# lionnus/I-ViT

Measured on AMD Instinct MI355X. Metric: images/sec DeiT-B INT8 @batch256, 1→8 MI355X; % INT8 MFMA peak, higher is better.
Workload: dtype int8; 1 GPU; DeiT-B INT8 integer-only forward, batch 256 per GPU, 224x224; global_batch=256, parallelism=dp1, launch=hip-graph replay, bitwidth=8, activation_ranges=power-of-two, operators=I-ViT (IVITIntLayerNorm, Shiftmax, ShiftGELU)

## Files before the change

i-vit_amd/csrc/check_resources.py:

```python
#!/usr/bin/env python3
import re
import sys

GUARDED = ("gemm_i8_wreg_kernel", "gemm_i8_pers_kernel")
FIELDS = {"VGPRs": r"\bVGPRs: (\d+)", "AGPRs": r"AGPRs: (\d+)", "Scratch": r"ScratchSize \[bytes/lane\]: (\d+)",
          "Occupancy": r"Occupancy \[waves/SIMD\]: (\d+)", "VGPRSpill": r"VGPRs Spill: (\d+)", "SGPRSpill": r"SGPRs Spill: (\d+)",
          "LDS": r"LDS Size \[bytes/block\]: (\d+)"}


def parse(text):
    kernels, cur = {}, None
    for line in text.splitlines():
        m = re.search(r"Function Name: (\S+)", line)
        if m:
            cur = kernels.setdefault(m.group(1), {})
            continue
        if cur is None:
            continue
        for k, pat in FIELDS.items():
            m = re.search(pat, line)
            if m and k not in cur:
                cur[k] = int(m.group(1))
    return kernels


def occupancy_rules(path, what):
    kernels = parse(open(path, errors="replace").read())
    bad, seen = [], 0
    for name, r in sorted(kernels.items()):
        if what == "attention" and "attention_long_kernel" in name:
            m = re.search(r"attention_long_kernelILi(\d+)ELb([01])ELi(\d+)ELi(\d+)E", name)
            occ, need_no_scratch = int(m.group(4)) // 256, True
        elif what == "attention" and "attention_cls_kernel" in name:
            occ, need_no_scratch = 3, True
        elif what == "attention":
            m = re.search(r"attention_kernelILi(\d+)ELi(\d+)ELi(\d+)ELb([01])E", name)
            if not m:
                continue
            occ, need_no_scratch = int(m.group(3)), m.group(4) == "0"
        elif what == "swin":
            if "window_attention_long_kernel" in name:
                occ, need_no_scratch = 2, True
            elif "window_attention_kernel" in name:
                occ, need_no_scratch = 4, True
            else:
                m = re.search(r"layernorm_i16_i8_tiled(_compat)?_kernelILi(\d+)ELi(\d+)E", name)
                if not m:
                    continue
                occ, need_no_scratch = (3 if m.group(1) and int(m.group(3)) >= 2 else 4), True
        elif "head_topk_kernel" in name:
            occ, need_no_scratch = 8, True
        else:
            m = re.search(r"layernorm_i8_stream_kernelILi(\d+)ELi(\d+)ELi(\d+)ELb([01])ELi(\d+)E", name)
            if not m:
                continue
            occ = int(m.group(5))
            need_no_scratch = m.group(4) == "0" or int(m.group(2)) == 3
        seen += 1
        ok = r.get("Occupancy", 0) >= occ and (r.get("Scratch") == 0 and r.get("VGPRSpill", 0) == 0 or not need_no_scratch)
        print(("ok   " if ok else "FAIL ") + f"{name}: VGPR {r.get('VGPRs')}, scratch {r.get('Scratch')}, occupancy {r.get('Occupancy')} (launcher assumes {occ}"
              f"{', no scratch' if need_no_scratch else ''})")
        if not ok:
            bad.append(name)
    if seen == 0:
        print("check_resources: no", what, "kernel found in", path)
        return 1
    if bad:
        print("check_resources: occupancy / scratch assumption of the launchers violated:", ", ".join(bad))
        return 1
    return 0


def main(path):
    kernels = parse(open(path, errors="replace").read())
    bad, seen = [], 0
    for name, r in sorted(kernels.items()):
        if not any(g in name for g in GUARDED):
            continue
        seen += 1
        regs = r.get("VGPRs", 0) + r.get("AGPRs", 0)
        line = (f"{name}: VGPR+AGPR {regs}, scratch {r.get('Scratch')}, VGPR spill {r.get('VGPRSpill')}, "
                f"SGPR spill {r.get('SGPRSpill')}, occupancy {r.get('Occupancy')}, LDS {r.get('LDS')}")
        ok = (r.get("Scratch") == 0 and r.get("VGPRSpill") == 0 and regs <= 256 and r.get("Occupancy", 0) >= 2
              and r.get("LDS", 0) <= 81920)
        print(("ok   " if ok else "FAIL ") + line)
        if not ok:
            bad.append(name)
    if seen == 0:
        print("check_resources: no guarded kernel found in", path)
        return 1
    if bad:
        print("check_resources: register / scratch budget of the inline-asm GEMM kernels violated:", ", ".join(bad))
        return 1
    return 0


if __name__ == "__main__":
    sys.exit(occupancy_rules(sys.argv[1], sys.argv[2]) if len(sys.argv) > 2 else main(sys.argv[1]))
```

i-vit_amd/csrc/gemm.hip:

```cpp
#include <type_traits>
#include "gemm_common.h"

namespace {

template <int EPI>
__global__ __launch_bounds__(NT) void gemm_i8_kernel(GemmArgs g)
{
    __shared__ __attribute__((aligned(16))) char smem[SMEM_BYTES + BN * 8];

    const int nblk = g.tiles_m * g.tiles_n;
    const int bid = blockIdx.x;
    const int q8 = nblk >> 3, r8 = nblk & 7, xcd = bid & 7;
    const int lid = (xcd < r8 ? xcd * (q8 + 1) : r8 * (q8 + 1) + (xcd - r8) * q8) + (bid >> 3);
    const int tm = lid / g.tiles_n, tn = lid - tm * g.tiles_n;
    const int m0 = tm * BM, n0 = tn * BN;

    const int tid = threadIdx.x;
    const int lane = tid & 63, wave = tid >> 6;
    const int wm = wave >> 1, wn = wave & 1;
    const int h = lane >> 5, l31 = lane & 31;
    if constexpr (EPI != EPI_I32 && EPI != EPI_RQ16 && EPI != EPI_RQ16_RES16) fill_rq_table(g, smem + SMEM_BYTES, n0, BN, tid);

    const int srow = tid >> 2, sc = tid & 3;
    const int8_t* ap[2];
// ... 862 lines not shown
                acc[ii] = *reinterpret_cast<const v4i*>(bias + 16 * i + 4 * g4);
#pragma unroll
                for (int ks = 0; ks < SK_MAXK / 32; ++ks)
                    if (ks < nks)
                        acc[ii] = __builtin_amdgcn_mfma_i32_16x16x32_i8(*reinterpret_cast<const long*>(smem + ((size_t)(i * nks + ks) * 64 + lane) * 8),
                                                                         bf[ks], acc[ii], 0, 0, 0);
            }
            int b[4][4];
            unsigned unc = 0;
#pragma unroll
            for (int ii = 0; ii < 4; ++ii) {
                const int i = min(i0 + ii, nsub - 1);
#pragma unroll
                for (int r = 0; r < 4; ++r) {
                    const float2 lh = lohi[16 * i + 4 * g4 + r];
                    const float a = (float)acc[ii][r];
                    const int tl = __float_as_int(__builtin_fmaf(a, lh.x, 12582912.0f));
                    const int th = __float_as_int(__builtin_fmaf(a, lh.y, 12582912.0f));
                    asm("v_sad_u32 %0, %1, %2, %3" : "=v"(unc) : "v"(tl), "v"(th), "v"(unc));
                    b[ii][r] = clamp_i32(tl, 0x4B400000 - 128, 0x4B400000 + 127);
                }
            }
            if (__builtin_amdgcn_ballot_w64(unc != 0) != 0) {
#pragma unroll
                for (int ii = 0; ii < 4; ++ii) {
                    const int c0 = 16 * min(i0 + ii, nsub - 1) + 4 * g4;
#pragma unroll
                    for (int r = 0; r < 4; ++r) {
                        const double tq = (double)acc[ii][r] * dyadic_mult(g.m[c0 + r], g.e[c0 + r]) + IVIT_MAGIC;
                        b[ii][r] = clamp_i32((int)(unsigned)__double_as_longlong(tq), -128, 127);
                    }
                }
            }
            unsigned D[4];
#pragma unroll
            for (int ii = 0; ii < 4; ++ii)
                D[ii] = __builtin_amdgcn_perm((unsigned)b[ii][1], (unsigned)b[ii][0], 0x0c0c0400u) |
                        __builtin_amdgcn_perm((unsigned)b[ii][3], (unsigned)b[ii][2], 0x04000c0cu);
            typedef unsigned v2u __attribute__((ext_vector_type(2)));
            const v2u ab = __builtin_amdgcn_permlane32_swap(D[0], D[2], false, false);
            const v2u cd = __builtin_amdgcn_permlane32_swap(D[1], D[3], false, false);
            const v2u ac = __builtin_amdgcn_permlane16_swap(ab.x, cd.x, false, false);
            const v2u bd = __builtin_amdgcn_permlane16_swap(ab.y, cd.y, false, false);
            const int ci = i0 + g4;
            if (ci < nsub && t < g.M) {
                const int4 v = make_int4((int)ac.x, (int)ac.y, (int)bd.x, (int)bd.y);
                if constexpr (EPI == EPI_QKV) *reinterpret_cast<int4*>(out + coff[4 * ci] + qrow_off) = v;
                else *reinterpret_cast<int4*>(out + (int64_t)t * g.ldo + 16 * ci) = v;
            }
        }
    }
}

template <int EPI>
int launch_gemm(GemmArgs& g, const char* name, ivit_stream_t stream, int qkv_planes = 3)
{
    IVIT_REQUIRE(g.A && g.W && g.out, "%s: NULL operand", name);
    IVIT_REQUIRE(g.M > 0 && g.N > 0 && g.K > 0, "%s: empty problem M=%d N=%d K=%d", name, g.M, g.N, g.K);
    IVIT_REQUIRE(g.K % BK == 0, "%s: K=%d must be a multiple of %d", name, g.K, BK);
    IVIT_REQUIRE(g.lda >= g.K && g.ldw >= g.K && g.lda % 16 == 0 && g.ldw % 16 == 0,
                 "%s: lda=%lld ldw=%lld must be >= K and multiples of 16", name, (long long)g.lda, (long long)g.ldw);
    IVIT_REQUIRE(((uintptr_t)g.A % 16 == 0) && ((uintptr_t)g.W % 16 == 0) && ((uintptr_t)g.out % 16 == 0),
                 "%s: operands must be 16-byte aligned", name);
    if (EPI == EPI_I32 || EPI == EPI_RQ16 || EPI == EPI_RQ16_RES16) {
        IVIT_REQUIRE(g.N % 4 == 0 && g.ldo % 4 == 0 && g.ldo >= g.N, "%s: N=%d ldo=%lld must be multiples of 4", name,
                     g.N, (long long)g.ldo);
        if (EPI == EPI_RQ16 || EPI == EPI_RQ16_RES16)
            IVIT_REQUIRE(g.m && g.e && ((uintptr_t)g.m % 16 == 0) && ((uintptr_t)g.e % 16 == 0) && ((uintptr_t)g.out % 8 == 0),
                         "%s: requantiser tables missing or misaligned", name);
    } else {
        IVIT_REQUIRE(g.m && g.e, "%s: NULL requantiser table", name);
        IVIT_REQUIRE(((uintptr_t)g.bias % 16 == 0), "%s: bias must be 16-byte aligned", name);
        IVIT_REQUIRE(g.N % 16 == 0, "%s: N=%d must be a multiple of 16", name, g.N);
        IVIT_REQUIRE(((uintptr_t)g.m % 16 == 0) && ((uintptr_t)g.e % 16 == 0), "%s: m/e tables must be 16-byte aligned",
                     name);
    }
    if (EPI == EPI_RQ || EPI == EPI_RESID)
        IVIT_REQUIRE(g.ldo >= g.N && g.ldo % 16 == 0, "%s: ldo=%lld must be >= N and a multiple of 16", name,
                     (long long)g.ldo);
    if (EPI == EPI_RESID)
        IVIT_REQUIRE(g.res && g.ldr >= g.N && g.ldr % 16 == 0 && ((uintptr_t)g.res % 16 == 0),
                     "%s: residual operand missing or misaligned", name);
    if (EPI == EPI_RESID16 || EPI == EPI_RQ16_RES16)
        IVIT_REQUIRE(g.res && g.ldr >= g.N && g.ldr % 8 == 0 && ((uintptr_t)g.res % 16 == 0) && g.ldo >= g.N && g.ldo % 8 == 0,
                     "%s: 16-bit residual / output rows must be 16-byte aligned (ld multiples of 8 elements)", name);
    if (EPI == EPI_QKV) {
        IVIT_REQUIRE(g.tokens > 0 && g.heads > 0 && g.head_dim > 0 && g.head_dim % 16 == 0,
                     "%s: bad head geometry tokens=%d heads=%d head_dim=%d", name, g.tokens, g.heads, g.head_dim);
        IVIT_REQUIRE((int64_t)g.M * g.N < 2147483648ll, "%s: q/k/v output of %lld bytes exceeds the 2 GiB the 32-bit head-major offsets cover",
                     name, (long long)g.M * g.N);
        IVIT_REQUIRE(g.N == qkv_planes * g.heads * g.head_dim && g.M % g.tokens == 0,
                     "%s: N=%d != %d*heads*head_dim or M=%d %% tokens=%d != 0", name, g.N, qkv_planes, g.M, g.tokens);
    }
#if IVIT_LAB
    g.stamp = reinterpret_cast<unsigned long long*>(g_stamp_buf);
#endif
    const bool blocks = g.a_blocks || g.w_blocks;
    if constexpr (EPI == EPI_RQ || EPI == EPI_QKV) {
        if (!blocks && !g.w_frags && !g.out_blocks && !g.lut && g.M >= 8192 && g.K >= 32 && g.K <= SK_MAXK && g.K % 32 == 0 && g.N >= 16 &&
            g.N <= SK_MAXN && g.N % 16 == 0 && g.lda % 16 == 0 && g.ldw % 8 == 0 && ((uintptr_t)g.A % 16 == 0) && ((uintptr_t)g.W % 8 == 0) &&
            ((uintptr_t)g.out % 16 == 0) && (EPI == EPI_QKV || g.ldo % 16 == 0) && (EPI != EPI_QKV || g.head_dim % 16 == 0) && (int64_t)g.M * (EPI == EPI_QKV ? g.N : g.ldo) < 4294967296ll &&
            !g_force_small && !(IVIT_LAB && (g_debug_flags2 & (1 << 20)))) {
            const int nstrips = (g.M + 15) >> 4;
            const int grid = (nstrips + SK_WPB - 1) / SK_WPB < 512 ? (nstrips + SK_WPB - 1) / SK_WPB : 512;
            const bool any_k = IVIT_LAB && (g_debug_flags2 & (1 << 21));
            if (g.K == 128 && !any_k) hipLaunchKernelGGL((gemm_i8_skinny_kernel<EPI, 4>), dim3(grid), dim3(SK_NT), 0, ivit_stream(stream), g);
// ... 40 lines not shown
                    default: break;
                }
            }
#endif
            if (g.w_frags == 2) {
                if constexpr (EPI != EPI_RQ16_RES16) {
                    IVIT_REQUIRE(((int64_t)g.M + 16) * (EPI == EPI_QKV ? g.N : g.ldo) < 4294967296ll &&
                                     (EPI != EPI_RESID || ((int64_t)g.M + 16) * g.ldr < 4294967296ll),
                                 "%s: IVIT_W_FRAGS16 addresses its output (and residual) with 32-bit offsets: operand of 4 GiB or more", name);
#if IVIT_LAB
                    if constexpr (EPI == EPI_RQ || EPI == EPI_RESID) {
                        if ((g_debug_flags2 & 256) && g.stamp) {
                            if (EPI == EPI_RESID && g.res_f32) hipLaunchKernelGGL((gemm_i8_wreg_kernel<EPI, 16 | 2048 | 4096, true>), grid, dim3(BIG_NT), 0, ivit_stream(stream), g);
                            else hipLaunchKernelGGL((gemm_i8_wreg_kernel<EPI, 16 | 2048, true>), grid, dim3(BIG_NT), 0, ivit_stream(stream), g);
                            IVIT_CHECK_LAUNCH(name);
                        }
                    }
#endif
                    if constexpr (EPI == EPI_RESID) {
                        if (g.res_f32) {
                            hipLaunchKernelGGL((gemm_i8_wreg_kernel<EPI, 4096, true>), grid, dim3(BIG_NT), 0, ivit_stream(stream), g);
                            IVIT_CHECK_LAUNCH(name);
                        }
                    }
                    hipLaunchKernelGGL((gemm_i8_wreg_kernel<EPI, 0, true>), grid, dim3(BIG_NT), 0, ivit_stream(stream), g);
                    IVIT_CHECK_LAUNCH(name);
                } else {
                    IVIT_REQUIRE(false, "%s: IVIT_W_FRAGS16 has no 16-bit epilogue; pack the weights with ivit_pack_weight_frags_i8", name);
                }
            }
            hipLaunchKernelGGL((gemm_i8_wreg_kernel<EPI>), grid, dim3(BIG_NT), 0, ivit_stream(stream), g);
            IVIT_CHECK_LAUNCH(name);
        }
    }
    if constexpr (EPI != EPI_I32 && EPI != EPI_RQ16 && EPI != EPI_RQ16_RES16) {
        if (g.M >= 2048 && g.N >= BCH && !g_force_small) {
            g.stagger = (g_debug_flags & 64) ? 0 : 512;
            g.tiles_m = (g.M + BTOK - 1) / BTOK;
            g.tiles_n = (g.N + BCH - 1) / BCH;
            const int ntiles = g.tiles_m * g.tiles_n;
            const bool one_per_cu = (g_debug_flags & 4096) != 0;
            const int SLOTS = (one_per_cu || (g_debug_flags & 67108864)) ? 256 : 512;
            const int rounds = ntiles / SLOTS, R = ntiles - rounds * SLOTS;
            const bool split = R > 0 && !(g_debug_flags & 134217728) &&
                               ((g_debug_flags & 2048) ? 2 * R <= SLOTS : 2 * R <= 256) && !one_per_cu;
            g.split_from = split ? rounds * SLOTS : ntiles;
            g.cu_turns = (g_debug_flags & 32768) ? 1 : 0;
            g.stagger_units = (g_debug_flags >> 16) & 63;
            const int grid = rounds > 0 ? SLOTS : (split ? 2 * R : R);
            hipLaunchKernelGGL((gemm_i8_pers_kernel<EPI>), dim3(grid), dim3(BIG_NT), one_per_cu ? 20480 : 0, ivit_stream(stream), g);
            IVIT_CHECK_LAUNCH(name);
        }
    }
    g.tiles_m = (g.M + BM - 1) / BM;
    g.tiles_n = (g.N + BN - 1) / BN;
    hipLaunchKernelGGL(gemm_i8_kernel<EPI>, dim3(g.tiles_m * g.tiles_n), dim3(NT), 0, ivit_stream(stream), g);
    IVIT_CHECK_LAUNCH(name);
}

__global__ __launch_bounds__(256) void pack_weight_frags_kernel(const int8_t* W, int64_t ldw, int N, int K, int8_t* dst)
{
    const int c16 = K >> 4, n64 = (N + 63) & ~63;
    const int64_t total = (int64_t)n64 * c16;
    for (int64_t q = (int64_t)blockIdx.x * 256 + threadIdx.x; q < total; q += (int64_t)gridDim.x * 256) {
        const int n = (int)(q / c16), k = (int)(q - (int64_t)n * c16) << 4;
        int4 v = make_int4(0, 0, 0, 0);
        if (n < N) v = *reinterpret_cast<const int4*>(W + (int64_t)n * ldw + k);
        const int64_t off = ((int64_t)(n >> 6) * (K >> 6) + (k >> 6)) * 4096 + ((((n >> 5) & 1) * 2 + ((k >> 5) & 1)) * 2 + ((k >> 4) & 1)) * 512 + (n & 31) * 16;
        *reinterpret_cast<int4*>(dst + off) = v;
    }
}

__global__ __launch_bounds__(256) void pack_weight_frags16_kernel(const int8_t* W, int64_t ldw, int N, int K, int8_t* dst)
{
    const int c16 = K >> 4, n64 = (N + 63) & ~63;
    const int64_t total = (int64_t)n64 * c16;
    for (int64_t q = (int64_t)blockIdx.x * 256 + threadIdx.x; q < total; q += (int64_t)gridDim.x * 256) {
        const int n = (int)(q / c16), k = (int)(q - (int64_t)n * c16) << 4;
        int4 v = make_int4(0, 0, 0, 0);
        if (n < N) v = *reinterpret_cast<const int4*>(W + (int64_t)n * ldw + k);
        const int64_t off = ((int64_t)(n >> 6) * (K >> 6) + (k >> 6)) * 4096 + ((n >> 4) & 3) * 1024 + ((k >> 4) & 3) * 256 + (n & 15) * 16;
        *reinterpret_cast<int4*>(dst + off) = v;
    }
}

}

IVIT_EXPORT int ivit_pack_weight_frags16_i8(const int8_t* W, int64_t ldw, int N, int K, int8_t* dst, ivit_stream_t stream)
{
    IVIT_REQUIRE(W && dst && N > 0 && K > 0 && K % 64 == 0 && ldw >= K && ldw % 16 == 0 && ((uintptr_t)W % 16 == 0) && ((uintptr_t)dst % 16 == 0),
                 "ivit_pack_weight_frags16_i8: bad operand (K must be a multiple of 64, rows 16-byte aligned)");
    const int64_t total = (int64_t)((N + 63) & ~63) * (K >> 4);
    const int grid = (int)((total + 255) / 256 < 4096 ? (total + 255) / 256 : 4096);
    hipLaunchKernelGGL(pack_weight_frags16_kernel, dim3(grid), dim3(256), 0, ivit_stream(stream), W, ldw, N, K, dst);
    IVIT_CHECK_LAUNCH("ivit_pack_weight_frags16_i8");
}

IVIT_EXPORT int ivit_pack_weight_frags_i8(const int8_t* W, int64_t ldw, int N, int K, int8_t* dst, ivit_stream_t stream)
{
    IVIT_REQUIRE(W && dst && N > 0 && K > 0 && K % 64 == 0 && ldw >= K && ldw % 16 == 0 && ((uintptr_t)W % 16 == 0) && ((uintptr_t)dst % 16 == 0),
                 "ivit_pack_weight_frags_i8: bad operand (K must be a multiple of 64, rows 16-byte aligned)");
    const int64_t total = (int64_t)((N + 63) & ~63) * (K >> 4);
    const int grid = (int)((total + 255) / 256 < 4096 ? (total + 255) / 256 : 4096);
    hipLaunchKernelGGL(pack_weight_frags_kernel, dim3(grid), dim3(256), 0, ivit_stream(stream), W, ldw, N, K, dst);
    IVIT_CHECK_LAUNCH("ivit_pack_weight_frags_i8");
}
// ... 222 lines not shown
```

i-vit_amd/csrc/gemm_common.h:

```cpp
#pragma once
#include <type_traits>

#include "common.h"

#if IVIT_LAB
extern bool g_force_small;
extern void* g_stamp_buf;
extern int g_debug_flags;
extern int g_debug_flags2;
#else
constexpr bool g_force_small = false;
constexpr int g_debug_flags = 0;
constexpr int g_debug_flags2 = 0;
#endif

namespace {

constexpr int BM = 128;
constexpr int BN = 128;
constexpr int BK = 64;
constexpr int NT = 256;
constexpr int STAGE_BYTES = (BM + BN) * BK;
constexpr int W_OFF = BM * BK;
constexpr int SMEM_BYTES = 2 * STAGE_BYTES;
// ... 345 lines not shown
                    for (int r = 0; r < 4; ++r) {
                        const double t = (double)acc[i][jb + j][r] * Mc[r] + IVIT_MAGIC;
                        b[j][r] = clamp_i32((int)(unsigned)__double_as_longlong(t), -128, 127);
                    }
            }
#pragma unroll
            for (int j = 0; j < 4; ++j) {
                const int tl_ = 16 * (jb + j) + l15;
                const unsigned w01 = __builtin_amdgcn_perm((unsigned)b[j][1], (unsigned)b[j][0], 0x0c0c0400u);
                const unsigned w23 = __builtin_amdgcn_perm((unsigned)b[j][3], (unsigned)b[j][2], 0x04000c0cu);
                *reinterpret_cast<unsigned*>(smem + tl_ * CSS + cl) = w01 | w23;
            }
        }
        __builtin_amdgcn_sched_barrier(0);
    }
    epilogue_phase2<EPI, 16 * NJ, NTHREADS, CH, Hook>(g, smem, m0, n0, tid, hook, lut_lds);
}

IVIT_DEV void residual_chunk_f32(int (&v)[4], const int4& res, float Mf_main, float Mf_res, float magic_v)
{
    const int rr[4] = {res.x, res.y, res.z, res.w};
#pragma unroll
    for (int d = 0; d < 4; ++d) {
        unsigned o[4];
#pragma unroll
        for (int bb = 0; bb < 4; ++bb) {
            const float kf = (float)(int)(int8_t)(v[d] >> (8 * bb));
            const float xf = (float)(int)(int8_t)(rr[d] >> (8 * bb));
            float f1, f2;
            asm("v_fma_f32 %0, %1, %2, %3" : "=v"(f1) : "v"(kf), "s"(Mf_main), "v"(magic_v));
            asm("v_fma_f32 %0, %1, %2, %3" : "=v"(f2) : "v"(xf), "s"(Mf_res), "v"(magic_v));
            o[bb] = (unsigned)clamp_i32((int)((unsigned)__float_as_int(f1) + (unsigned)__float_as_int(f2) - 2u * 0x4B400000u), -128, 127);
        }
        v[d] = (int)(__builtin_amdgcn_perm(o[1], o[0], 0x0c0c0400u) | __builtin_amdgcn_perm(o[3], o[2], 0x04000c0cu));
    }
}

IVIT_DEV void residual_chunk_f64(int (&v)[4], const int4& res, double M_main, double M_res)
{
    const int rr[4] = {res.x, res.y, res.z, res.w};
#pragma unroll
    for (int d = 0; d < 4; ++d) {
        int o[4];
#pragma unroll
        for (int bb = 0; bb < 4; ++bb) {
            const int k3 = (int)(int8_t)(v[d] >> (8 * bb));
            const int xr = (int)(int8_t)(rr[d] >> (8 * bb));
            o[bb] = clamp_i32(requant_exact(k3, M_main) + requant_exact(xr, M_res), -128, 127);
        }
        v[d] = pack4_i8(o[0], o[1], o[2], o[3]);
    }
}

template <int EPI, int NJ, int ABL, typename Hook>
IVIT_DEV void epilogue_direct_16(v4i (&acc)[4][NJ], const GemmArgs& g, const char* rq_lds, int m0, int n0, int wch, int g4, int l15,
                                 const Hook& hook, const unsigned char* lut_lds, unsigned long long* st = nullptr)
{
    static_assert(NJ % 4 == 0 && (EPI == EPI_RQ || EPI == EPI_RESID || EPI == EPI_QKV), "direct epilogue: int8 outputs");
    __builtin_amdgcn_s_setprio(2);
    hook.issue();
    const unsigned rq_a = lds_addr(rq_lds) + 8u * (unsigned)(wch + 4 * g4);
    const int ncol = n0 + wch;
    const bool col_ok = ncol < g.N;
    const int c = ncol + 16 * g4;
    constexpr int NB = NJ / 4;
    unsigned D[NB][4][4];
    int4 rv[EPI == EPI_RESID ? NB : 1][4];
    v4f lhbuf[2][2];
    lds_read16_async(lhbuf[0][0], rq_a);
    lds_read16_async(lhbuf[0][1], rq_a + 16u);
#pragma unroll
    for (int bi = 0; bi < NB; ++bi) {
        const int jb = 4 * bi;
#pragma unroll
        for (int i = 0; i < 4; ++i) {
            const int sidx = jb + i;
            v4f& lh01 = lhbuf[sidx & 1][0];
            v4f& lh23 = lhbuf[sidx & 1][1];
            lds_wait(lh01, lh23);
            if (sidx + 1 < NJ) {
                const unsigned nxt = rq_a + 8u * (unsigned)(16 * ((i + 1) & 3));
                lds_read16_async(lhbuf[(sidx + 1) & 1][0], nxt);
                lds_read16_async(lhbuf[(sidx + 1) & 1][1], nxt + 16u);
            }
            const float lo[4] = {lh01.x, lh01.z, lh23.x, lh23.z};
            const float hi[4] = {lh01.y, lh01.w, lh23.y, lh23.w};
            int b[4][4];
            unsigned unc = 0;
#pragma unroll
            for (int j = 0; j < 4; ++j)
#pragma unroll
                for (int r = 0; r < 4; ++r) {
                    const float a = (float)acc[i][jb + j][r];
                    const int tl = __float_as_int(__builtin_fmaf(a, lo[r], 12582912.0f));
                    const int th = __float_as_int(__builtin_fmaf(a, hi[r], 12582912.0f));
                    asm("v_sad_u32 %0, %1, %2, %3" : "=v"(unc) : "v"(tl), "v"(th), "v"(unc));
                    b[j][r] = clamp_i32(tl, 0x4B400000 - 128, 0x4B400000 + 127);
                }
            if (__builtin_amdgcn_ballot_w64(unc != 0) != 0) {
                const int c0 = min(ncol + 16 * i + 4 * g4, g.N - 4);
                const uint4 m4 = *reinterpret_cast<const uint4*>(g.m + c0);
                const int4 e4 = *reinterpret_cast<const int4*>(g.e + c0);
                const double Mc[4] = {dyadic_mult(m4.x, e4.x), dyadic_mult(m4.y, e4.y), dyadic_mult(m4.z, e4.z), dyadic_mult(m4.w, e4.w)};
#pragma unroll
                for (int j = 0; j < 4; ++j)
#pragma unroll
// ... 302 lines not shown
```

i-vit_amd/csrc/rowops.hip:

```cpp
#include <limits.h>

#include "common.h"
#include "rowsum.h"

#if IVIT_LAB
int g_ln_wave_per_row = 0;
int g_ln_ablate = 0;
int g_ln_stream_cfg = 0;
unsigned long long* g_ln_stamps = nullptr;
#else
constexpr int g_ln_wave_per_row = 0;
constexpr int g_ln_ablate = 0;
constexpr int g_ln_stream_cfg = 0;
#endif

namespace {

typedef float v2f __attribute__((ext_vector_type(2)));

constexpr int NT = 256;
constexpr int WPB = NT / 64;

IVIT_DEV int sx8(int v, int byte) { return (int)(int8_t)(v >> (8 * byte)); }

// ... 974 lines not shown
    if (blockIdx.x == 0 && threadIdx.x == 0)
        for (int64_t t = n & ~(int64_t)3; t < n; ++t) out[t] = (int8_t)quant_sym_i8(x[t], inv_scale);
}

__global__ __launch_bounds__(NT) void quantize_i32_kernel(const float* x, int32_t* out, int64_t n, float inv_scale, float lo,
                                                          float hi)
{
    for (int64_t i = (int64_t)blockIdx.x * NT + threadIdx.x; i < n; i += (int64_t)gridDim.x * NT) {
        float v = rintf(inv_scale * x[i]);
        v = fminf(fmaxf(v, lo), hi);
        out[i] = (int32_t)fminf(v, 2147483520.0f);
    }
}

__global__ __launch_bounds__(NT) void patchify_kernel(const float* img, int8_t* A, int64_t lda, int batch, int chans,
                                                      int hw, int patch, float inv_scale)
{
    const int g = hw / patch;
    const int pw4 = patch >> 2;
    const int64_t total = (int64_t)batch * chans * hw * (hw >> 2);
    if (total < 2147483648ll) {
        const unsigned w4 = (unsigned)(hw >> 2), tot = (unsigned)total;
        for (unsigned q = blockIdx.x * NT + threadIdx.x; q < tot; q += gridDim.x * NT) {
            const unsigned r = q / w4, x4 = q - r * w4;
            const unsigned r2 = r / (unsigned)hw, y = r - r2 * (unsigned)hw;
            const unsigned b = r2 / (unsigned)chans, c = r2 - b * (unsigned)chans;
            const float4 v = *reinterpret_cast<const float4*>(img + (size_t)r * hw + 4 * x4);
            const unsigned px = x4 / (unsigned)pw4, kw = (x4 - px * pw4) * 4;
            const unsigned py = y / (unsigned)patch, kh = y - py * patch;
            const int64_t row = ((int64_t)b * g + py) * g + px;
            const unsigned col = (c * patch + kh) * patch + kw;
            *reinterpret_cast<int*>(A + row * lda + col) = pack4(quant_sym_i8(v.x, inv_scale), quant_sym_i8(v.y, inv_scale),
                                                                 quant_sym_i8(v.z, inv_scale), quant_sym_i8(v.w, inv_scale));
        }
        return;
    }
    for (int64_t q = (int64_t)blockIdx.x * NT + threadIdx.x; q < total; q += (int64_t)gridDim.x * NT) {
        int x4 = (int)(q % (hw >> 2));
        int64_t r = q / (hw >> 2);
        int y = (int)(r % hw);
        r /= hw;
        int c = (int)(r % chans);
        int b = (int)(r / chans);
        float4 v = *reinterpret_cast<const float4*>(img + (((int64_t)b * chans + c) * hw + y) * hw + 4 * x4);
        int px = x4 / pw4, kw = (x4 - px * pw4) * 4;
        int py = y / patch, kh = y - py * patch;
        int64_t row = ((int64_t)b * g + py) * g + px;
        int col = (c * patch + kh) * patch + kw;
        *reinterpret_cast<int*>(A + row * lda + col) = pack4(quant_sym_i8(v.x, inv_scale), quant_sym_i8(v.y, inv_scale),
                                                             quant_sym_i8(v.z, inv_scale), quant_sym_i8(v.w, inv_scale));
    }
}

__global__ __launch_bounds__(NT) void patchify_u8_kernel(const uint8_t* img, int8_t* A, int64_t lda, int batch, int chans, int hw,
                                                         int patch, const int8_t* lut)
{
    __shared__ int8_t s_lut[4 * 256];
    for (int i = threadIdx.x; i < chans * 256; i += NT) s_lut[i] = lut[i];
    __syncthreads();
    const int g = hw / patch;
    const int pw4 = patch >> 2;
    const int64_t total = (int64_t)batch * chans * hw * (hw >> 2);
    for (int64_t q = (int64_t)blockIdx.x * NT + threadIdx.x; q < total; q += (int64_t)gridDim.x * NT) {
        int x4 = (int)(q % (hw >> 2));
        int64_t r = q / (hw >> 2);
        int y = (int)(r % hw);
        r /= hw;
        int c = (int)(r % chans);
        int b = (int)(r / chans);
        const unsigned v = *reinterpret_cast<const unsigned*>(img + (((int64_t)b * chans + c) * hw + y) * hw + 4 * x4);
        const int8_t* t = s_lut + 256 * c;
        int px = x4 / pw4, kw = (x4 - px * pw4) * 4;
        int py = y / patch, kh = y - py * patch;
        int64_t row = ((int64_t)b * g + py) * g + px;
        int col = (c * patch + kh) * patch + kw;
        *reinterpret_cast<int*>(A + row * lda + col) = pack4(t[v & 255], t[(v >> 8) & 255], t[(v >> 16) & 255], t[v >> 24]);
    }
}

__global__ __launch_bounds__(NT) void embed_kernel(const int8_t* patch, const int16_t* pos_add, const int8_t* cls_row,
                                                   double Mq, int8_t* out, int batch, int tokens, int C)
{
    const int cd = C >> 2;
    const int64_t total = (int64_t)batch * tokens * cd;
    for (int64_t q = (int64_t)blockIdx.x * NT + threadIdx.x; q < total; q += (int64_t)gridDim.x * NT) {
        int d = (int)(q % cd);
        int64_t r = q / cd;
        int tok = (int)(r % tokens);
        int b = (int)(r / tokens);
        int res;
        if (tok == 0) {
            res = *reinterpret_cast<const int*>(cls_row + 4 * d);
        } else {
            int w = *reinterpret_cast<const int*>(patch + ((int64_t)b * (tokens - 1) + tok - 1) * C + 4 * d);
            const int16_t* pa = pos_add + (int64_t)tok * C + 4 * d;
            int o[4];
#pragma unroll
            for (int c = 0; c < 4; ++c) o[c] = clamp_i32(requant_exact(sx8(w, c), Mq) + (int)pa[c], -128, 127);
            res = pack4(o[0], o[1], o[2], o[3]);
        }
        *reinterpret_cast<int*>(out + ((int64_t)b * tokens + tok) * C + 4 * d) = res;
    }
}

__global__ __launch_bounds__(NT) void embed16_kernel(const int16_t* patch, const int32_t* pos_add, const int16_t* cls_row,
                                                     double Mq, int16_t* out, int batch, int tokens, int C)
{
    const int cd = C >> 2;
    const int64_t total = (int64_t)batch * tokens * cd;
    for (int64_t q = (int64_t)blockIdx.x * NT + threadIdx.x; q < total; q += (int64_t)gridDim.x * NT) {
        const int d = (int)(q % cd);
        const int64_t r = q / cd;
        const int tok = (int)(r % tokens);
        const int b = (int)(r / tokens);
        int2 res;
        if (tok == 0) {
            res = *reinterpret_cast<const int2*>(cls_row + 4 * d);
        } else {
            const int2 w = *reinterpret_cast<const int2*>(patch + ((int64_t)b * (tokens - 1) + tok - 1) * C + 4 * d);
            const int4 pa = *reinterpret_cast<const int4*>(pos_add + (int64_t)tok * C + 4 * d);
            const int k[4] = {(int)(int16_t)w.x, w.x >> 16, (int)(int16_t)w.y, w.y >> 16};
            const int p4[4] = {pa.x, pa.y, pa.z, pa.w};
            int o[4];
#pragma unroll
            for (int c = 0; c < 4; ++c) o[c] = clamp_i32(requant_exact(k[c], Mq) + p4[c], -32768, 32767);
            res.x = (o[0] & 0xffff) | (o[1] << 16);
            res.y = (o[2] & 0xffff) | (o[3] << 16);
        }
        *reinterpret_cast<int2*>(out + ((int64_t)b * tokens + tok) * C + 4 * d) = res;
    }
}

__global__ __launch_bounds__(NT) void head_argmax_kernel(const int32_t* acc, const float* s_acc, int batch, int N,
                                                         float* logits, int32_t* top1)
{
    const int lane = threadIdx.x & 63, wave = __builtin_amdgcn_readfirstlane(threadIdx.x >> 6);
    for (int row = blockIdx.x * WPB + wave; row < batch; row += gridDim.x * WPB) {
        float best = -__builtin_inff();
        int bi = 0x7fffffff;
        for (int n = lane; n < N; n += 64) {
            float v = (float)acc[(int64_t)row * N + n] * s_acc[n];
            if (logits) logits[(int64_t)row * N + n] = v;
            if (v > best) { best = v; bi = n; }
        }
#pragma unroll
        for (int o = 32; o > 0; o >>= 1) {
            float ob = __shfl_xor(best, o);
            int oi = __shfl_xor(bi, o);
            if (ob > best || (ob == best && oi < bi)) { best = ob; bi = oi; }
        }
        if (lane == 0) top1[row] = bi;
    }
}

// ... 589 lines not shown

IVIT_EXPORT int ivit_shiftmax_i8(const int8_t* x, int64_t ldx, int rows, int L, float s, int8_t* out, int64_t ldo,
                                 ivit_stream_t stream)
{
    return launch_shiftmax<int8_t>("ivit_shiftmax_i8", x, ldx, rows, L, s, out, ldo, stream);
}

IVIT_EXPORT int ivit_shiftmax_i32_i8(const int32_t* x, int64_t ldx, int rows, int L, float s, int8_t* out, int64_t ldo,
                                     ivit_stream_t stream)
{
    return launch_shiftmax<int32_t>("ivit_shiftmax_i32_i8", x, ldx, rows, L, s, out, ldo, stream);
}

IVIT_EXPORT int ivit_minmax_f32(const float* x, int64_t n, float* out_min_max, ivit_stream_t stream)
{
    IVIT_REQUIRE(x && out_min_max && n > 0, "ivit_minmax_f32: bad operand");
    IVIT_REQUIRE(((uintptr_t)out_min_max % 4 == 0) && ((uintptr_t)x % 4 == 0), "ivit_minmax_f32: misaligned");
    hipStream_t st = ivit_stream(stream);
    unsigned* keys = reinterpret_cast<unsigned*>(out_min_max);
    hipLaunchKernelGGL(minmax_init_kernel, dim3(1), dim3(1), 0, st, keys);
    hipLaunchKernelGGL(minmax_kernel, dim3(ew_grid(n) < 2048 ? ew_grid(n) : 2048), dim3(NT), 0, st, x, n, keys);
    hipLaunchKernelGGL(minmax_finish_kernel, dim3(1), dim3(1), 0, st, keys);
    IVIT_CHECK_LAUNCH("ivit_minmax_f32");
}

IVIT_EXPORT int ivit_quantize_input_f32_i8(const float* x, int8_t* out, int64_t n, float inv_scale,
                                           ivit_stream_t stream)
{
    IVIT_REQUIRE(x && out && n > 0, "ivit_quantize_input_f32_i8: bad operand");
    IVIT_REQUIRE(((uintptr_t)x % 16 == 0) && ((uintptr_t)out % 4 == 0), "ivit_quantize_input_f32_i8: misaligned");
    hipLaunchKernelGGL(quantize_kernel, dim3(ew_grid(n / 4 + 1)), dim3(NT), 0, ivit_stream(stream), x, out, n,
                       inv_scale);
    IVIT_CHECK_LAUNCH("ivit_quantize_input_f32_i8");
}

IVIT_EXPORT int ivit_quantize_input_f32_i32(const float* x, int32_t* out, int64_t n, float inv_scale, int bits,
                                            ivit_stream_t stream)
{
    IVIT_REQUIRE(x && out && n > 0 && bits >= 2 && bits <= 32, "ivit_quantize_input_f32_i32: bad operand");
    const float lo = -__builtin_ldexpf(1.0f, bits - 1), hi = __builtin_ldexpf(1.0f, bits - 1) - 1.0f;
    hipLaunchKernelGGL(quantize_i32_kernel, dim3(ew_grid(n)), dim3(NT), 0, ivit_stream(stream), x, out, n, inv_scale, lo, hi);
    IVIT_CHECK_LAUNCH("ivit_quantize_input_f32_i32");
}

static int launch_patchify(const char* who, const float* img, int8_t* A, int64_t lda, int batch, int chans, int hw, int patch,
                           float inv_scale, ivit_stream_t stream)
{
    IVIT_REQUIRE(img && A && batch > 0 && chans > 0, "%s: bad operand", who);
    IVIT_REQUIRE(patch > 0 && patch % 4 == 0 && hw % patch == 0, "%s: hw=%d patch=%d", who, hw, patch);
    IVIT_REQUIRE(lda >= (int64_t)chans * patch * patch && lda % 4 == 0, "%s: lda=%lld too small or not a multiple of 4", who,
                 (long long)lda);
    IVIT_REQUIRE(((uintptr_t)img % 16 == 0) && ((uintptr_t)A % 4 == 0), "%s: misaligned", who);
    const int64_t total = (int64_t)batch * chans * hw * (hw / 4);
    hipLaunchKernelGGL(patchify_kernel, dim3(ew_grid(total)), dim3(NT), 0, ivit_stream(stream), img, A, lda, batch, chans,
                       hw, patch, inv_scale);
    IVIT_CHECK_LAUNCH(who);
}

IVIT_EXPORT int ivit_quantize_patchify_f32_i8(const float* img, int8_t* A, int batch, int chans, int hw, int patch,
                                              float inv_scale, ivit_stream_t stream)
{
    return launch_patchify("ivit_quantize_patchify_f32_i8", img, A, (int64_t)chans * patch * patch, batch, chans, hw, patch,
                           inv_scale, stream);
}

IVIT_EXPORT int ivit_quantize_patchify_u8_i8(const uint8_t* img, int8_t* A, int64_t lda, int batch, int chans, int hw, int patch,
                                             const int8_t* lut, ivit_stream_t stream)
{
    IVIT_REQUIRE(img && A && lut && batch > 0 && chans > 0 && chans <= 4 && hw > 0 && patch > 0 && hw % patch == 0 && patch % 4 == 0,
                 "ivit_quantize_patchify_u8_i8: bad shape (up to 4 channels, hw %% patch == 0, patch %% 4 == 0)");
    IVIT_REQUIRE(lda >= (int64_t)chans * patch * patch && lda % 4 == 0 && ((uintptr_t)img % 4 == 0) && ((uintptr_t)A % 4 == 0),
                 "ivit_quantize_patchify_u8_i8: lda too small or misaligned operand");
    const int64_t total = (int64_t)batch * chans * hw * (hw / 4);
    hipLaunchKernelGGL(patchify_u8_kernel, dim3(ew_grid(total)), dim3(NT), 0, ivit_stream(stream), img, A, lda, batch, chans, hw,
                       patch, lut);
    IVIT_CHECK_LAUNCH("ivit_quantize_patchify_u8_i8");
}

IVIT_EXPORT int ivit_quantize_patchify_ld_f32_i8(const float* img, int8_t* A, int64_t lda, int batch, int chans, int hw,
                                                 int patch, float inv_scale, ivit_stream_t stream)
{
    return launch_patchify("ivit_quantize_patchify_ld_f32_i8", img, A, lda, batch, chans, hw, patch, inv_scale, stream);
}

IVIT_EXPORT int ivit_embed_assemble_i8(const int8_t* patch, const int16_t* pos_add, const int8_t* cls_row, uint32_t m,
                                       int32_t e, int8_t* out, int batch, int tokens, int C, ivit_stream_t stream)
{
    IVIT_REQUIRE(patch && pos_add && cls_row && out, "ivit_embed_assemble_i8: NULL operand");
    IVIT_REQUIRE(batch > 0 && tokens > 1 && C > 0 && C % 4 == 0, "ivit_embed_assemble_i8: bad shape");
    IVIT_REQUIRE(((uintptr_t)patch % 4 == 0) && ((uintptr_t)out % 4 == 0) && ((uintptr_t)cls_row % 4 == 0) &&
                     ((uintptr_t)pos_add % 8 == 0),
                 "ivit_embed_assemble_i8: misaligned");
    const double Mq = ivit_dyadic_to_double(m, e);
    IVIT_REQUIRE(Mq < 1048576.0, "ivit_embed_assemble_i8: requant multiplier too large");
    const int64_t total = (int64_t)batch * tokens * (C / 4);
    hipLaunchKernelGGL(embed_kernel, dim3(ew_grid(total)), dim3(NT), 0, ivit_stream(stream), patch, pos_add, cls_row,
                       Mq, out, batch, tokens, C);
    IVIT_CHECK_LAUNCH("ivit_embed_assemble_i8");
}

IVIT_EXPORT int ivit_embed_assemble_i16(const int16_t* patch, const int32_t* pos_add, const int16_t* cls_row, uint32_t m,
                                        int32_t e, int16_t* out, int batch, int tokens, int C, ivit_stream_t stream)
{
    IVIT_REQUIRE(patch && pos_add && cls_row && out, "ivit_embed_assemble_i16: NULL operand");
    IVIT_REQUIRE(batch > 0 && tokens > 1 && C > 0 && C % 4 == 0, "ivit_embed_assemble_i16: bad shape");
    IVIT_REQUIRE(((uintptr_t)patch % 8 == 0) && ((uintptr_t)out % 8 == 0) && ((uintptr_t)cls_row % 8 == 0) &&
                     ((uintptr_t)pos_add % 16 == 0),
                 "ivit_embed_assemble_i16: misaligned");
    const double Mq = ivit_dyadic_to_double(m, e);
    IVIT_REQUIRE(Mq < 32768.0, "ivit_embed_assemble_i16: requant multiplier too large");
    const int64_t total = (int64_t)batch * tokens * (C / 4);
    hipLaunchKernelGGL(embed16_kernel, dim3(ew_grid(total)), dim3(NT), 0, ivit_stream(stream), patch, pos_add, cls_row,
                       Mq, out, batch, tokens, C);
    IVIT_CHECK_LAUNCH("ivit_embed_assemble_i16");
}

IVIT_EXPORT int ivit_head_argmax(const int32_t* acc, const float* s_acc, int batch, int N, float* logits_f32,
                                 int32_t* top1, ivit_stream_t stream)
{
    IVIT_REQUIRE(acc && s_acc && top1 && batch > 0 && N > 0, "ivit_head_argmax: bad operand");
    hipLaunchKernelGGL(head_argmax_kernel, dim3(grid_for_rows(batch)), dim3(NT), 0, ivit_stream(stream), acc, s_acc,
                       batch, N, logits_f32, top1);
    IVIT_CHECK_LAUNCH("ivit_head_argmax");
}

namespace {
template <bool F32>
void launch_head_topk(int k, const int32_t* acc, const float* s_acc, const float* logits_in, int batch, int ld, int N,
                      float* logits_out, int32_t* topk, const int32_t* targets, uint64_t* hits, hipStream_t s)
{
    unsigned long long* h = reinterpret_cast<unsigned long long*>(hits);
    const dim3 grid(grid_for_rows(batch)), block(NT);
#define IVIT_TOPK_CASE(K) \
    case K: hipLaunchKernelGGL((head_topk_kernel<K, F32>), grid, block, 0, s, acc, s_acc, logits_in, batch, ld, N, logits_out, topk, targets, h); break;
    switch (k) {
        IVIT_TOPK_CASE(1) IVIT_TOPK_CASE(2) IVIT_TOPK_CASE(3) IVIT_TOPK_CASE(4)
        IVIT_TOPK_CASE(5) IVIT_TOPK_CASE(6) IVIT_TOPK_CASE(7) IVIT_TOPK_CASE(8)
    }
#undef IVIT_TOPK_CASE
}
static_assert(IVIT_TOPK_MAX == 8, "launch_head_topk instantiates k = 1..8");
}

IVIT_EXPORT int ivit_head_topk(const int32_t* acc, const float* s_acc, int batch, int ld, int N, int k, float* logits_f32,
                               int32_t* topk, const int32_t* targets, uint64_t* hits, ivit_stream_t stream)
{
    IVIT_REQUIRE(acc && s_acc && topk && batch > 0, "ivit_head_topk: bad operand");
    IVIT_REQUIRE(k >= 1 && k <= IVIT_TOPK_MAX && k <= N && N <= ld, "ivit_head_topk: bad k=%d / N=%d / ld=%d", k, N, ld);
// ... 106 lines not shown
```

Baseline: 40780 images/s.

## Add small-M split-K GEMM, banded patchify, and streamed embed assembly kernels

Adds a split-K MFMA GEMM path for M<=256 (e.g. the classifier head on CLS rows), where four waves each take a share of the K steps and partial sums are reduced through LDS. Adds a patchify kernel that stages one patch row band in LDS so each patch is written as contiguous 16-byte rows. Adds an embed-assembly kernel that streams 16-byte chunks, several per thread. All three target launch count and poorly coalesced memory traffic in small, bandwidth-bound stages, at the cost of more code paths, new guard conditions and extra resource checks.

```diff
diff --git a/i-vit_amd/csrc/check_resources.py b/i-vit_amd/csrc/check_resources.py
--- a/i-vit_amd/csrc/check_resources.py
+++ b/i-vit_amd/csrc/check_resources.py
@@ -48,6 +48,10 @@
                 if not m:
                     continue
                 occ, need_no_scratch = (3 if m.group(1) and int(m.group(3)) >= 2 else 4), True
+        elif "patchify_band_kernel" in name:
+            occ, need_no_scratch = 8, True
+        elif "embed_stream_kernel" in name:
+            occ, need_no_scratch = 6, True
         elif "head_topk_kernel" in name:
             occ, need_no_scratch = 8, True
         else:
@@ -75,6 +79,14 @@
     kernels = parse(open(path, errors="replace").read())
     bad, seen = [], 0
     for name, r in sorted(kernels.items()):
+        if "gemm_i8_small_m_kernel" in name:
+            seen += 1
+            ok = r.get("Scratch") == 0 and r.get("VGPRSpill") == 0 and r.get("Occupancy", 0) >= 2
+            print(("ok   " if ok else "FAIL ") + f"{name}: VGPR {r.get('VGPRs')}, AGPR {r.get('AGPRs')}, scratch {r.get('Scratch')}, "
+                  f"VGPR spill {r.get('VGPRSpill')}, occupancy {r.get('Occupancy')}, LDS {r.get('LDS')}")
+            if not ok:
+                bad.append(name)
+            continue
         if not any(g in name for g in GUARDED):
             continue
         seen += 1
diff --git a/i-vit_amd/csrc/gemm.hip b/i-vit_amd/csrc/gemm.hip
--- a/i-vit_amd/csrc/gemm.hip
+++ b/i-vit_amd/csrc/gemm.hip
@@ -938,6 +938,89 @@
     }
 }
 
+constexpr int SM_MAXM = 256, SM_NJ = 8, SM_ROWS = 16 * SM_NJ, SM_DEPTH = 4;
+
+struct SmFrag { v4i w, a[SM_NJ]; };
+
+template <int EPI>
+__global__ __launch_bounds__(NT) void gemm_i8_small_m_kernel(GemmArgs g)
+{
+    static_assert(EPI == EPI_RQ || EPI == EPI_RESID || EPI == EPI_I32, "small-M form: row-major int8 / int32 outputs");
+    __shared__ __attribute__((aligned(16))) v4i part[4][SM_NJ][64];
+    const int tid = threadIdx.x, lane = tid & 63, wave = __builtin_amdgcn_readfirstlane(tid >> 6);
+    const int l15 = lane & 15, g4 = lane >> 4;
+    const int n0 = blockIdx.x * 16, m0 = blockIdx.y * SM_ROWS;
+
+    const unsigned woff = (unsigned)min(n0 + l15, g.N - 1) * (unsigned)g.ldw + 16u * g4;
+    unsigned aoff[SM_NJ];
+#pragma unroll
+    for (int j = 0; j < SM_NJ; ++j) aoff[j] = (unsigned)min(m0 + 16 * j + l15, g.M - 1) * (unsigned)g.lda + 16u * g4;
+    auto load = [&](SmFrag& f, int s) {
+        const unsigned k = (unsigned)s * BK;
+        f.w = *reinterpret_cast<const v4i*>(g.W + (woff + k));
+#pragma unroll
+        for (int j = 0; j < SM_NJ; ++j) f.a[j] = *reinterpret_cast<const v4i*>(g.A + (aoff[j] + k));
+    };
+
+    const int nk = g.K / BK, cnt = (nk - wave + 3) >> 2;
+    SmFrag f[SM_DEPTH];
+#pragma unroll
+    for (int d = 0; d < SM_DEPTH; ++d)
+        if (d < cnt) load(f[d], wave + 4 * d);
+    const int t = m0 + tid;
+    const bool row_ok = tid < SM_ROWS && t < g.M;
+    int4 rv = make_int4(0, 0, 0, 0);
+    if constexpr (EPI == EPI_RESID)
+        if (row_ok) rv = *reinterpret_cast<const int4*>(g.res + (int64_t)t * g.ldr + n0);
+
+    v4i acc[SM_NJ];
+#pragma unroll
+    for (int j = 0; j < SM_NJ; ++j) acc[j] = v4i{0, 0, 0, 0};
+    for (int i = 0; i < cnt; i += SM_DEPTH) {
+#pragma unroll
+        for (int d = 0; d < SM_DEPTH; ++d) {
+            if (i + d < cnt) {
+#pragma unroll
+                for (int j = 0; j < SM_NJ; ++j) acc[j] = __builtin_amdgcn_mfma_i32_16x16x64_i8(f[d].w, f[d].a[j], acc[j], 0, 0, 0);
+                if (i + d + SM_DEPTH < cnt) load(f[d], wave + 4 * (i + d + SM_DEPTH));
+            }
+        }
+    }
+#pragma unroll
+    for (int j = 0; j < SM_NJ; ++j) part[wave][j][lane] = acc[j];
+    __syncthreads();
+    if (!row_ok) return;
+
+    const int j = tid >> 4, r15 = tid & 15;
+    int s[16];
+#pragma unroll
+    for (int c = 0; c < 4; ++c) {
+        v4i v = part[0][j][16 * c + r15];
+#pragma unroll
+        for (int w = 1; w < 4; ++w) v += part[w][j][16 * c + r15];
+        if (g.bias != nullptr) v += *reinterpret_cast<const v4i*>(g.bias + min(n0 + 4 * c, g.N - 4));
+#pragma unroll
+        for (int r = 0; r < 4; ++r) s[4 * c + r] = v[r];
+    }
+    if constexpr (EPI == EPI_I32) {
+        int32_t* out = reinterpret_cast<int32_t*>(g.out) + (int64_t)t * g.ldo + n0;
+#pragma unroll
+        for (int c = 0; c < 4; ++c)
+            if (n0 + 4 * c < g.N) *reinterpret_cast<v4i*>(out + 4 * c) = v4i{s[4 * c], s[4 * c + 1], s[4 * c + 2], s[4 * c + 3]};
+    } else {
+        int v[4];
+#pragma unroll
+        for (int c = 0; c < 4; ++c) {
+            const uint4 m4 = *reinterpret_cast<const uint4*>(g.m + n0 + 4 * c);
+            const int4 e4 = *reinterpret_cast<const int4*>(g.e + n0 + 4 * c);
+            v[c] = pack4_i8(requant_literal_i8(s[4 * c], dyadic_mult(m4.x, e4.x)), requant_literal_i8(s[4 * c + 1], dyadic_mult(m4.y, e4.y)),
+                            requant_literal_i8(s[4 * c + 2], dyadic_mult(m4.z, e4.z)), requant_literal_i8(s[4 * c + 3], dyadic_mult(m4.w, e4.w)));
+        }
+        if constexpr (EPI == EPI_RESID) residual_chunk_f64(v, rv, g.M_main, g.M_res);
+        *reinterpret_cast<int4*>(reinterpret_cast<int8_t*>(g.out) + (int64_t)t * g.ldo + n0) = make_int4(v[0], v[1], v[2], v[3]);
+    }
+}
+
 template <int EPI>
 int launch_gemm(GemmArgs& g, const char* name, ivit_stream_t stream, int qkv_planes = 3)
 {
@@ -1084,6 +1167,14 @@
             IVIT_CHECK_LAUNCH(name);
         }
     }
+    if constexpr (EPI == EPI_RQ || EPI == EPI_RESID || EPI == EPI_I32) {
+        if (g.M <= SM_MAXM && !blocks && !g.w_frags && !g.out_blocks && !g.lut && (EPI == EPI_I32 || g.N % 16 == 0) && (g.N + 15) / 16 <= 65535 &&
+            (int64_t)g.M * g.lda < (1ll << 31) && (int64_t)g.N * g.ldw < (1ll << 31) && (g.bias == nullptr || (uintptr_t)g.bias % 16 == 0) &&
+            !g_force_small) {
+            hipLaunchKernelGGL(gemm_i8_small_m_kernel<EPI>, dim3((g.N + 15) / 16, (g.M + SM_ROWS - 1) / SM_ROWS), dim3(NT), 0, ivit_stream(stream), g);
+            IVIT_CHECK_LAUNCH(name);
+        }
+    }
     g.tiles_m = (g.M + BM - 1) / BM;
     g.tiles_n = (g.N + BN - 1) / BN;
     hipLaunchKernelGGL(gemm_i8_kernel<EPI>, dim3(g.tiles_m * g.tiles_n), dim3(NT), 0, ivit_stream(stream), g);
diff --git a/i-vit_amd/csrc/gemm_common.h b/i-vit_amd/csrc/gemm_common.h
--- a/i-vit_amd/csrc/gemm_common.h
+++ b/i-vit_amd/csrc/gemm_common.h
@@ -421,6 +421,12 @@
     }
 }
 
+IVIT_DEV int requant_literal_i8(int acc, double M)
+{
+    const double t = (double)acc * M + IVIT_MAGIC;
+    return clamp_i32((int)(unsigned)__double_as_longlong(t), -128, 127);
+}
+
 template <int EPI, int NJ, int ABL, typename Hook>
 IVIT_DEV void epilogue_direct_16(v4i (&acc)[4][NJ], const GemmArgs& g, const char* rq_lds, int m0, int n0, int wch, int g4, int l15,
                                  const Hook& hook, const unsigned char* lut_lds, unsigned long long* st = nullptr)
diff --git a/i-vit_amd/csrc/rowops.hip b/i-vit_amd/csrc/rowops.hip
--- a/i-vit_amd/csrc/rowops.hip
+++ b/i-vit_amd/csrc/rowops.hip
@@ -1050,6 +1050,55 @@
     }
 }
 
+static inline unsigned small_div_magic(unsigned d) { return 0x80000000u / d; }
+IVIT_DEV unsigned small_div(unsigned n, unsigned magic) { return __umulhi(2u * n + 1u, magic); }
+
+struct PatchifyArgs {
+    const float* img;
+    int8_t* A;
+    int64_t lda;
+    unsigned chans, hw, patch, g;
+    unsigned items;
+    unsigned w4, pw4;
+    unsigned m_w4, m_pw4, m_cw, m_r16;
+    unsigned r16, lrow;
+    float inv_scale;
+};
+constexpr int PF_U = 4;
+
+__global__ __launch_bounds__(NT) void patchify_band_kernel(const PatchifyArgs a)
+{
+    extern __shared__ __attribute__((aligned(16))) int8_t s_band[];
+    const unsigned py = blockIdx.x, b = blockIdx.y;
+    const float* src = a.img + ((size_t)b * a.chans * a.hw + (size_t)py * a.patch) * a.hw;
+    const unsigned cstep = a.hw * a.hw - a.patch * a.hw;
+    for (unsigned q0 = threadIdx.x; q0 < a.items; q0 += PF_U * NT) {
+        float4 v[PF_U];
+#pragma unroll
+        for (int u = 0; u < PF_U; ++u) {
+            const unsigned q = q0 + u * NT;
+            if (q < a.items) v[u] = *reinterpret_cast<const float4*>(src + (small_div(q, a.m_cw) * cstep + 4 * q));
+        }
+#pragma unroll
+        for (int u = 0; u < PF_U; ++u) {
+            const unsigned q = q0 + u * NT;
+            if (q < a.items) {
+                const unsigned r = small_div(q, a.m_w4), x4 = q - r * a.w4;
+                const unsigned px = small_div(x4, a.m_pw4), kw4 = x4 - px * a.pw4;
+                *reinterpret_cast<int*>(s_band + px * a.lrow + r * a.patch + 4 * kw4) =
+                    pack4(quant_sym_i8(v[u].x, a.inv_scale), quant_sym_i8(v[u].y, a.inv_scale), quant_sym_i8(v[u].z, a.inv_scale),
+                          quant_sym_i8(v[u].w, a.inv_scale));
+            }
+        }
+    }
+    __syncthreads();
+    int8_t* dst = a.A + ((int64_t)b * a.g + py) * a.g * a.lda;
+    for (unsigned t = threadIdx.x; t < a.g * a.r16; t += NT) {
+        const unsigned px = small_div(t, a.m_r16), c16 = t - px * a.r16;
+        *reinterpret_cast<int4*>(dst + (px * (unsigned)a.lda + 16 * c16)) = *reinterpret_cast<const int4*>(s_band + px * a.lrow + 16 * c16);
+    }
+}
+
 __global__ __launch_bounds__(NT) void patchify_u8_kernel(const uint8_t* img, int8_t* A, int64_t lda, int batch, int chans, int hw,
                                                          int patch, const int8_t* lut)
 {
@@ -1098,6 +1147,51 @@
             res = pack4(o[0], o[1], o[2], o[3]);
         }
         *reinterpret_cast<int*>(out + ((int64_t)b * tokens + tok) * C + 4 * d) = res;
+    }
+}
+
+constexpr int EM_U = 4;
+
+__global__ __launch_bounds__(NT) void embed_stream_kernel(const int8_t* patch, const int16_t* pos_add, const int8_t* cls_row, double Mq,
+                                                          int8_t* out, unsigned tokens, unsigned C)
+{
+    const unsigned n16 = (tokens - 1) * (C >> 4);
+    const int8_t* src = patch + (size_t)blockIdx.y * n16 * 16;
+    int8_t* dst = out + (size_t)blockIdx.y * tokens * C + C;
+    const int16_t* pos = pos_add + C;
+    const unsigned j0 = blockIdx.x * (EM_U * NT) + threadIdx.x;
+    int4 w[EM_U], p0[EM_U], p1[EM_U];
+#pragma unroll
+    for (int u = 0; u < EM_U; ++u) {
+        const unsigned j = j0 + u * NT;
+        if (j < n16) {
+            w[u] = *reinterpret_cast<const int4*>(src + 16 * j);
+            p0[u] = *reinterpret_cast<const int4*>(pos + 16 * j);
+            p1[u] = *reinterpret_cast<const int4*>(pos + 16 * j + 8);
+        }
+    }
+    if (blockIdx.x == 0)
+        for (unsigned t = threadIdx.x; t < (C >> 4); t += NT)
+            *reinterpret_cast<int4*>(dst - C + 16 * t) = *reinterpret_cast<const int4*>(cls_row + 16 * t);
+#pragma unroll
+    for (int u = 0; u < EM_U; ++u) {
+        const unsigned j = j0 + u * NT;
+        if (j < n16) {
+            const int wv[4] = {w[u].x, w[u].y, w[u].z, w[u].w};
+            const int pv[8] = {p0[u].x, p0[u].y, p0[u].z, p0[u].w, p1[u].x, p1[u].y, p1[u].z, p1[u].w};
+            int r[4];
+#pragma unroll
+            for (int d = 0; d < 4; ++d) {
+                int o[4];
+#pragma unroll
+                for (int c = 0; c < 4; ++c) {
+                    const int pa = (c & 1) ? pv[2 * d + (c >> 1)] >> 16 : (int)(int16_t)pv[2 * d + (c >> 1)];
+                    o[c] = clamp_i32(requant_exact(sx8(wv[d], c), Mq) + pa, -128, 127);
+                }
+                r[d] = pack4(o[0], o[1], o[2], o[3]);
+            }
+            *reinterpret_cast<int4*>(dst + 16 * j) = make_int4(r[0], r[1], r[2], r[3]);
+        }
     }
 }
 
@@ -1793,6 +1887,19 @@
                  (long long)lda);
     IVIT_REQUIRE(((uintptr_t)img % 16 == 0) && ((uintptr_t)A % 4 == 0), "%s: misaligned", who);
     const int64_t total = (int64_t)batch * chans * hw * (hw / 4);
+    const int g = hw / patch;
+    const int64_t band_lds = (int64_t)g * ((int64_t)chans * patch * patch + 16);
+    if (((uintptr_t)A % 16 == 0) && lda % 16 == 0 && band_lds <= 65536 && batch <= 65535 && (int64_t)chans * hw * hw < (1ll << 30) &&
+        (int64_t)g * lda < (1ll << 31) && !(g_ln_ablate & (1 << 27))) {
+        PatchifyArgs a{img, A, lda, (unsigned)chans, (unsigned)hw, (unsigned)patch, (unsigned)g};
+        a.w4 = hw / 4, a.pw4 = patch / 4, a.items = chans * patch * a.w4, a.r16 = chans * patch * patch / 16;
+        a.m_w4 = small_div_magic(a.w4), a.m_pw4 = small_div_magic(a.pw4), a.m_cw = small_div_magic(patch * a.w4);
+        a.m_r16 = small_div_magic(a.r16);
+        a.lrow = chans * patch * patch + 16;
+        a.inv_scale = inv_scale;
+        hipLaunchKernelGGL(patchify_band_kernel, dim3(g, batch), dim3(NT), (size_t)band_lds, ivit_stream(stream), a);
+        IVIT_CHECK_LAUNCH(who);
+    }
     hipLaunchKernelGGL(patchify_kernel, dim3(ew_grid(total)), dim3(NT), 0, ivit_stream(stream), img, A, lda, batch, chans,
                        hw, patch, inv_scale);
     IVIT_CHECK_LAUNCH(who);
@@ -1835,6 +1942,13 @@
     const double Mq = ivit_dyadic_to_double(m, e);
     IVIT_REQUIRE(Mq < 1048576.0, "ivit_embed_assemble_i8: requant multiplier too large");
     const int64_t total = (int64_t)batch * tokens * (C / 4);
+    if (C % 16 == 0 && (((uintptr_t)patch | (uintptr_t)pos_add | (uintptr_t)cls_row | (uintptr_t)out) % 16 == 0) && batch <= 65535 &&
+        (int64_t)tokens * C < (1ll << 31) && !(g_ln_ablate & (1 << 27))) {
+        const unsigned n16 = (unsigned)(tokens - 1) * (unsigned)(C / 16);
+        hipLaunchKernelGGL(embed_stream_kernel, dim3((n16 + EM_U * NT - 1) / (EM_U * NT), batch), dim3(NT), 0, ivit_stream(stream), patch,
+                           pos_add, cls_row, Mq, out, (unsigned)tokens, (unsigned)C);
+        IVIT_CHECK_LAUNCH("ivit_embed_assemble_i8");
+    }
     hipLaunchKernelGGL(embed_kernel, dim3(ew_grid(total)), dim3(NT), 0, ivit_stream(stream), patch, pos_add, cls_row,
                        Mq, out, batch, tokens, C);
     IVIT_CHECK_LAUNCH("ivit_embed_assemble_i8");
```

After: 41170 images/s (median of 6 runs). About the same (+1.0%).
